# razayunus/ManhattanSLAM

Measured on AMD Instinct MI355X. Metric: RGB-D frames/sec at 640x480 (ORB+surfel front end), higher is better.
Workload: dtype u8/i32 (ORB)/f32+f64 (surfel)

## Files before the change

manhattanslam_amd/csrc/msl_orb.hip:

```cpp

#include "msl_orb_dev.h"

#include <type_traits>

#include <cfloat>
#include <cmath>
#include <cstdlib>

using namespace msl;
using namespace msl::orb;

namespace {

__constant__ int8_t c_pattern[1024] = {
#include "../../include/msl_orb_pattern.inc"
};

__device__ __forceinline__ const uint8_t *level_ptr(const OrbDev &P, int frame, int l, int &pitch) {
    if (l == 0) { pitch = (int)P.inRowStride; return P.in + (size_t)frame * P.inFrameStride; }
    pitch = P.lv[l].pitch;
    return P.pyr + (size_t)frame * P.pyrStride + P.lv[l].off;
}

__device__ __forceinline__ bool xcd_item(int nx, int ny, int &x, int &y) {
    const unsigned g = blockIdx.x, C = gridDim.x >> 3;
    const unsigned v = (g & 7u) * C + (g >> 3);
    if (v >= (unsigned)nx * (unsigned)ny) return false;
    x = (int)(v % (unsigned)nx); y = (int)(v / (unsigned)nx);
    return true;
}
inline unsigned xcd_grid1(long long items) { return (unsigned)(8 * ((items + 7) / 8)); }

__global__ __launch_bounds__(256) void k_resize(OrbDev P, int l) {
    const int frame = blockIdx.z;
    const LevelDev &D = P.lv[l];
    const int dx = blockIdx.x * 64 + (threadIdx.x & 63);
    const int dy = blockIdx.y * 4 + (threadIdx.x >> 6);
    if (dx >= D.w || dy >= D.h) return;
    int sp;
    const uint8_t *src = level_ptr(P, frame, l - 1, sp);
    const ResizeTap tx = P.taps[D.xtabOff + dx], ty = P.taps[D.ytabOff + dy];
    const uint8_t *r0 = src + (size_t)ty.s0 * sp, *r1 = src + (size_t)ty.s1 * sp;
    const int h0 = r0[tx.s0] * tx.c0 + r0[tx.s1] * tx.c1;
    const int h1 = r1[tx.s0] * tx.c0 + r1[tx.s1] * tx.c1;
    int v = (((ty.c0 * (h0 >> 4)) >> 16) + ((ty.c1 * (h1 >> 4)) >> 16) + 2) >> 2;
    v = min(max(v, 0), 255);
    P.pyr[(size_t)frame * P.pyrStride + D.off + (size_t)dy * D.pitch + dx] = (uint8_t)v;
}

__global__ __launch_bounds__(256) void k_pyramid(OrbDev P) {
    extern __shared__ uint8_t s_pyr[];
    int tileI, frame;
    if (!xcd_item(P.pyrTX * P.pyrTY, P.nFrames, tileI, frame)) return;
    const int ti = tileI % P.pyrTX, tj = tileI / P.pyrTX;
    const int L = P.nlevels;
    PyrRange rx = P.pyrX[ti], ry = P.pyrY[tj];
    int sx0 = rx.needLo, sy0 = ry.needLo, sw = rx.needHi - rx.needLo, sh = ry.needHi - ry.needLo;
    int spitch = (sw + 3) & ~3;
    {
        int pitch;
        const uint8_t *img = level_ptr(P, frame, 0, pitch);
        const int nw = spitch >> 2, imgW = P.lv[0].w;
        const unsigned m = ((1u << 22) + nw - 1) / nw;
        for (int i = threadIdx.x; i < nw * sh; i += 256) {
            const int r = (int)__umulhi((unsigned)i << 10, m), q = i - r * nw;
            const int x = sx0 + 4 * q;
            const uint8_t *src = img + (unsigned)((sy0 + r) * pitch + x);
            unsigned v = 0;
            if (x + 3 < imgW) __builtin_memcpy(&v, src, 4);
            else
                for (int e = 0; e < 4 && x + e < imgW; e++) v |= (unsigned)src[e] << (8 * e);
            reinterpret_cast<unsigned *>(s_pyr)[i] = v;
        }
    }
    __syncthreads();
    for (int l = 1; l < L; l++) {
        const LevelDev &D = P.lv[l];
        const uint8_t *src = s_pyr + (((l - 1) & 1) ? P.pyrBuf0 : 0u);
        uint8_t *dst = s_pyr + ((l & 1) ? P.pyrBuf0 : 0u);
        rx = P.pyrX[l * P.pyrTX + ti]; ry = P.pyrY[l * P.pyrTY + tj];
        const int dx0 = rx.needLo, dy0 = ry.needLo, dw = rx.needHi - rx.needLo, dh = ry.needHi - ry.needLo;
        uint8_t *out = P.pyr + (size_t)frame * P.pyrStride + D.off;
        const unsigned m = ((1u << 22) + dw - 1) / dw;
        for (int i = threadIdx.x; i < dw * dh; i += 256) {
            const int r = (int)__umulhi((unsigned)i << 10, m), c = i - r * dw;
            const int dx = dx0 + c, dy = dy0 + r;
            const ResizeTap tx = P.taps[D.xtabOff + dx], ty = P.taps[D.ytabOff + dy];
            const uint8_t *r0 = src + (ty.s0 - sy0) * spitch - sx0, *r1 = src + (ty.s1 - sy0) * spitch - sx0;
            const int h0 = r0[tx.s0] * tx.c0 + r0[tx.s1] * tx.c1;
            const int h1 = r1[tx.s0] * tx.c0 + r1[tx.s1] * tx.c1;
            int v = (((ty.c0 * (h0 >> 4)) >> 16) + ((ty.c1 * (h1 >> 4)) >> 16) + 2) >> 2;
            v = min(max(v, 0), 255);
            dst[i] = (uint8_t)v;
            if (dx >= rx.ownLo && dx < rx.ownHi && dy >= ry.ownLo && dy < ry.ownHi) out[(size_t)dy * D.pitch + dx] = (uint8_t)v;
        }
        sx0 = dx0; sy0 = dy0; sw = dw; sh = dh; spitch = dw;
        __syncthreads();
    }
}

typedef short s16x2 __attribute__((ext_vector_type(2)));
__device__ __forceinline__ s16x2 pk_min(s16x2 a, s16x2 b) { return __builtin_elementwise_min(a, b); }
__device__ __forceinline__ s16x2 pk_max(s16x2 a, s16x2 b) { return __builtin_elementwise_max(a, b); }
__device__ __forceinline__ int fast_score16(const uint8_t *t, int tp) {
    const int v = t[0];
    const int ring[16] = {t[3 * tp], t[3 * tp + 1], t[2 * tp + 2], t[tp + 3], t[3], t[-tp + 3], t[-2 * tp + 2], t[-3 * tp + 1],
                          t[-3 * tp], t[-3 * tp - 1], t[-2 * tp - 2], t[-tp - 3], t[-3], t[tp - 3], t[2 * tp - 2], t[3 * tp - 1]};
    s16x2 x[16], lo2[16], lo4[16];
#pragma unroll
    for (int k = 0; k < 16; k++) { const int d = v - ring[k]; x[k] = (s16x2){(short)d, (short)-d}; }
#pragma unroll
    for (int k = 0; k < 16; k++) lo2[k] = pk_min(x[k], x[(k + 1) & 15]);
#pragma unroll
    for (int k = 0; k < 16; k++) lo4[k] = pk_min(lo2[k], lo2[(k + 2) & 15]);
    s16x2 a = (s16x2){(short)-256, (short)-256};
#pragma unroll
    for (int k = 0; k < 16; k++) a = pk_max(a, pk_min(pk_min(lo4[k], lo4[(k + 4) & 15]), x[(k + 8) & 15]));
    return max((int)a.x, (int)a.y) - 1;
}

__device__ __forceinline__ bool fast_candidate(const uint8_t *t, int tp, int th) {
    const int v = t[0];
    const int d0 = v - t[3 * tp], d8 = v - t[-3 * tp], d4 = v - t[3], d12 = v - t[-3];
    const int d2 = v - t[2 * tp + 2], d10 = v - t[-2 * tp - 2], d6 = v - t[-2 * tp + 2], d14 = v - t[2 * tp - 2];
    const bool bright = (d0 > th || d8 > th) && (d4 > th || d12 > th) && (d2 > th || d10 > th) && (d6 > th || d14 > th);
    const bool dark = (d0 < -th || d8 < -th) && (d4 < -th || d12 < -th) && (d2 < -th || d10 < -th) && (d6 < -th || d14 < -th);
    return bright || dark;
}

__global__ __launch_bounds__(256) void k_fast(OrbDev P) {
    __shared__ __attribute__((aligned(4))) uint8_t s_tile[(MAXCELL + 6) * (MAXCELL + 8)];
    __shared__ __attribute__((aligned(4))) uint8_t s_score[(MAXCELL + 2) * (MAXCELL + 2)];
    __shared__ unsigned s_bits[2][MAXCELL * MAXCELL / 32];
    __shared__ unsigned short s_list[MAXCELL * MAXCELL];
    __shared__ unsigned s_wave[17];
    __shared__ unsigned s_cnt[3];

    int cellI, frame;
    if (!xcd_item(P.cellsPerFrame, P.nFrames, cellI, frame)) return;
    const CellDev C = P.cells[cellI];
    const int tid = threadIdx.x;
    uint32_t *cnt_out = P.cellCnt + (size_t)frame * P.cellsPerFrame + cellI;
    const int cw = C.cw, ch = C.ch;
    if (cw <= 0 || ch <= 0) { if (tid == 0) *cnt_out = 0; return; }
    int pitch;
    const uint8_t *img = level_ptr(P, frame, C.level, pitch);

    const int tw = cw + 6, th = ch + 6, tp = (tw + 3) & ~3;
    const unsigned mCw = ((1u << 20) + cw - 1) / cw;
    {
        const int nw = tp >> 2;
        const unsigned mNw = ((1u << 20) + nw - 1) / nw;
        const uint8_t *src = img + (size_t)(C.y0 - 3) * pitch + (C.x0 - 3);
        for (int i = tid; i < nw * th; i += 256) {
            const int r = (int)(((unsigned)i * mNw) >> 20), q = i - r * nw;
            uint32_t w4;
            __builtin_memcpy(&w4, src + (size_t)r * pitch + 4 * q, 4);
            *reinterpret_cast<uint32_t *>(&s_tile[r * tp + 4 * q]) = w4;
        }
    }
    const int sp = cw + 2;
    for (int i = tid; i < (sp * (ch + 2) + 3) >> 2; i += 256) reinterpret_cast<uint32_t *>(s_score)[i] = 0u;
    if (tid < MAXCELL * MAXCELL / 32) { s_bits[0][tid] = 0; s_bits[1][tid] = 0; }
    if (tid < 3) s_cnt[tid] = 0;
    __syncthreads();
    const int npx = cw * ch;
    const int thQuick = min(P.iniTh, P.minTh);
    for (int i0 = 0; i0 < npx; i0 += 256) {
        const int i = i0 + tid;
        bool cand = false;
        if (i < npx) {
            const int r = (int)(((unsigned)i * mCw) >> 20), c = i - r * cw;
            cand = fast_candidate(&s_tile[(r + 3) * tp + c + 3], tp, thQuick);
        }
        const unsigned long long m = __ballot(cand);
        if (m) {
            unsigned base = 0;
            if ((tid & 63) == 0) base = atomicAdd(&s_cnt[2], (unsigned)__popcll(m));
            base = (unsigned)__builtin_amdgcn_readlane((int)base, 0);
            if (cand) s_list[base + __popcll(m & ((1ull << (tid & 63)) - 1ull))] = (unsigned short)i;
        }
    }
    __syncthreads();
    const int nlist = (int)s_cnt[2];
    for (int j = tid; j < nlist; j += 256) {
        const int i = s_list[j];
        const int r = (int)(((unsigned)i * mCw) >> 20), c = i - r * cw;
        const int s = fast_score16(&s_tile[(r + 3) * tp + c + 3], tp);
        s_score[(r + 1) * sp + c + 1] = (uint8_t)max(s, 0);
    }
    __syncthreads();
    unsigned c_ini = 0, c_min = 0;
    for (int j = tid; j < nlist; j += 256) {
        const int i = s_list[j];
        const int r = (int)(((unsigned)i * mCw) >> 20), c = i - r * cw;
        const uint8_t *q = &s_score[(r + 1) * sp + c + 1];
        const int s = q[0];
        if (s < thQuick) continue;
        const bool lm = s > q[-1] && s > q[1] && s > q[-sp - 1] && s > q[-sp] && s > q[-sp + 1] &&
                        s > q[sp - 1] && s > q[sp] && s > q[sp + 1];
        if (!lm) continue;
        if (s >= P.iniTh) { atomicOr(&s_bits[0][i >> 5], 1u << (i & 31)); c_ini++; }
        if (s >= P.minTh) { atomicOr(&s_bits[1][i >> 5], 1u << (i & 31)); c_min++; }
    }
    if (c_ini) atomicAdd(&s_cnt[0], c_ini);
    if (c_min) atomicAdd(&s_cnt[1], c_min);
    __syncthreads();
    const int sel = s_cnt[0] ? 0 : 1;
    const unsigned total = s_cnt[0] ? s_cnt[0] : s_cnt[1];
    if (tid == 0) *cnt_out = total;
    if (total == 0) return;
    uint32_t *out = P.cellKeys + (size_t)frame * P.keysPerFrame + C.keyOff;
    static_assert(MAXCELL * MAXCELL / 32 <= 256, "one bitmap word per thread");
    unsigned word = tid < MAXCELL * MAXCELL / 32 ? s_bits[sel][tid] : 0u;
    unsigned tot;
    unsigned pos = block_excl_scan((unsigned)__popc(word), s_wave, &tot);
    while (word) {
        const int i = tid * 32 + __builtin_ctz(word);
        word &= word - 1;
        const int r = (int)(((unsigned)i * mCw) >> 20), c = i - r * cw;
        const unsigned kx = C.x0 + c - 16, ky = C.y0 + r - 16;
        out[pos++] = kx | (ky << 12) | ((unsigned)s_score[(r + 1) * sp + c + 1] << 24);
    }
}

struct Rect { short x0, y0, x1, y1; };

__device__ __forceinline__ int quadrant(const Rect r, int x, int y) {
    const int mx = r.x0 + ((r.x1 - r.x0 + 1) >> 1), my = r.y0 + ((r.y1 - r.y0 + 1) >> 1);
    return (x < mx ? 0 : 1) + (y < my ? 0 : 2);
}
__device__ __forceinline__ Rect child_rect(const Rect r, int q) {
    const short mx = r.x0 + ((r.x1 - r.x0 + 1) >> 1), my = r.y0 + ((r.y1 - r.y0 + 1) >> 1);
    Rect c;
    c.x0 = (q & 1) ? mx : r.x0; c.x1 = (q & 1) ? r.x1 : mx;
    c.y0 = (q & 2) ? my : r.y0; c.y1 = (q & 2) ? r.y1 : my;
    return c;
}

#ifdef MSL_OCT_STAMPS
#define OCT_STAMP(P, level, frame, idx)                                                                                   \
    do {                                                                                                                  \
        const int i_ = (idx);                                                                                             \
        if ((level) == 0 && (frame) == 0 && threadIdx.x == 0 && i_ < 100) {                                               \
            unsigned long long *d_ = reinterpret_cast<unsigned long long *>(reinterpret_cast<unsigned char *>((P).err) + 128); \
            d_[2 * i_] = __builtin_amdgcn_s_memrealtime(); d_[2 * i_ + 1] = __builtin_amdgcn_s_memtime();                 \
        }                                                                                                                 \
    } while (0)
#else
#define OCT_STAMP(P, level, frame, idx) do { } while (0)
#endif
template <int KPT> struct OctKeys {
    static constexpr bool REG = KPT > 0;
    static constexpr int OCT_KPT = KPT > 0 ? KPT : 1;
    uint32_t key[OCT_KPT];
    unsigned node[OCT_KPT], quad[OCT_KPT];
    uint32_t *gkeys; uint16_t *gnode; unsigned n; int tid;
    unsigned per;
    template <typename F> __device__ __forceinline__ void for_each(F f) {
        if constexpr (REG) {
#pragma unroll
            for (int j = 0; j < OCT_KPT; j++) {
                const unsigned k = (unsigned)tid * per + (unsigned)j;
                if ((unsigned)j < per && k < n) f(k, key[j], node[j], quad[j]);
            }
        } else {
            for (unsigned k = tid; k < n; k += OCT_NT) {
                unsigned nd = gnode[k], q = 0xFFFFFFFFu;
                const unsigned nd0 = nd;
                f(k, gkeys[k], nd, q);
                if (nd != nd0) gnode[k] = (uint16_t)nd;
            }
        }
    }
};

template <int KPT>
__device__ __forceinline__ void octree_body(const OrbDev &P, const LevelDev &G, OctKeys<KPT> &K, unsigned char *s_dyn, unsigned *s_wave, int *s_misc, int frame,
                                            int level) {
    constexpr bool REG = KPT > 0;
    constexpr int OCT_KPT = KPT > 0 ? KPT : 1;
    const int M = P.maxNode, tid = threadIdx.x, N = G.quota;
    const unsigned n = K.n;
    Rect *const s_rectB = reinterpret_cast<Rect *>(s_dyn);
    unsigned *const s_cntB = reinterpret_cast<unsigned *>(s_rectB + 2 * M);
    unsigned *const s_cc = s_cntB + 2 * M;
    short *const s_crankB = reinterpret_cast<short *>(s_cc + 4 * M);
    unsigned *const s_FG = reinterpret_cast<unsigned *>(s_crankB + 2 * M);
    unsigned short *const s_L = reinterpret_cast<unsigned short *>(s_FG + 4 * M);
    unsigned short *const s_order = s_L + M;
    unsigned short *const s_rankOf = s_order + M;
    int *nsel = P.nsel + frame * P.nlevels + level;
    uint32_t *sel = P.sel + ((size_t)frame * P.nlevels + level) * P.selCap;

    const unsigned lane = (unsigned)tid & 63u;
    auto hist_add = [&](unsigned *ctr, unsigned q) {
        unsigned long long todo = __ballot(q != 0xFFFFFFFFu);
        while (todo) {
            const unsigned leader = (unsigned)__builtin_ctzll(todo);
            const unsigned qq = (unsigned)__builtin_amdgcn_readlane((int)q, (int)leader);
            const unsigned long long mm = __ballot(q == qq);
            if (lane == leader) atomicAdd(&ctr[qq], (unsigned)__popcll(mm));
            todo &= ~mm;
        }
    };
    auto for_each_hist = [&](unsigned *ctr, auto f) {
// ... 571 lines not shown
    unsigned w = nib | ((unsigned)__builtin_amdgcn_update_dpp(0, (int)nib, 0x101, 0xF, 0xF, true) << 4);
    w |= (unsigned)__builtin_amdgcn_update_dpp(0, (int)w, 0x102, 0xF, 0xF, true) << 8;
    w |= (unsigned)__builtin_amdgcn_update_dpp(0, (int)w, 0x104, 0xF, 0xF, true) << 16;
    msl_keypoint *kp = P.kps + (size_t)frame * P.outCap + outIdx;
    uint32_t *dsc = (uint32_t *)(P.desc + ((size_t)frame * P.outCap + outIdx) * 32);
    if ((lane & 7) == 0) dsc[lane >> 3] = w;
    if (lane == 0) {
        float fx = (float)x, fy = (float)y;
        if (level != 0) { fx *= D.scale; fy *= D.scale; }
        kp->x = fx; kp->y = fy; kp->size = (float)D.patch; kp->angle = angle;
        kp->response = (float)score; kp->octave = level; kp->class_id = -1;
        if (P.frameOn) {
            const size_t o = (size_t)frame * P.outCap + outIdx;
            float ux = fx, uy = fy;
            if (P.fp.k1 != 0.0) undistort_point(P.fp, fx, fy, &ux, &uy);
            P.unXY[2 * o] = ux; P.unXY[2 * o + 1] = uy;
            const float d = *(const float *)((const uint8_t *)P.depth + (size_t)frame * P.depthFrameStride + (size_t)(int)fy * P.depthRowStride +
                                             sizeof(float) * (size_t)(int)fx);
            P.depthOut[o] = d > 0 ? d : -1.0f;
            P.uRight[o] = d > 0 ? ux - P.fp.bf / d : -1.0f;
            const int posX = (int)roundf((ux - P.fp.minX) * P.gridWInv), posY = (int)roundf((uy - P.fp.minY) * P.gridHInv);
            P.gridCell[o] = (posX < 0 || posX >= MSL_FRAME_GRID_COLS || posY < 0 || posY >= MSL_FRAME_GRID_ROWS) ? -1 : posX * MSL_FRAME_GRID_ROWS + posY;
        }
    }
}

const char *kKernelNames[MSL_ORB_NKERNELS] = {"k_pyramid", "k_fast", "k_octree", "k_blur", "k_describe", "copy"};

}

namespace msl {
namespace orb {

const char *kernel_name(int kid) { return kKernelNames[kid]; }

int allow_octree_lds(int octLds) {
    if (octLds <= 32 * 1024) return MSL_OK;
    MSL_HIP_TRY(hipFuncSetAttribute(reinterpret_cast<const void *>(k_octree<16>), hipFuncAttributeMaxDynamicSharedMemorySize, octLds));
    MSL_HIP_TRY(hipFuncSetAttribute(reinterpret_cast<const void *>(k_octree<32>), hipFuncAttributeMaxDynamicSharedMemorySize, octLds));
    return MSL_OK;
}

}
}

int orb_launch_pipeline(const OrbDev *dev, OrbLaunch *launch, const uint8_t *d_gray, size_t rowStride, size_t frameStride, int n,
                        msl_keypoint *d_kps, uint8_t *d_desc, int *d_nout, const FrameEpilogue *ep) {
    OrbLaunch &q = *launch;
    OrbDev P = *dev;
    P.in = d_gray; P.inRowStride = rowStride; P.inFrameStride = frameStride;
    P.kps = d_kps; P.desc = d_desc; P.nout = d_nout;
    P.frameOn = ep ? 1 : 0;
    P.nFrames = n;
    if (ep) {
        P.fp = ep->fp;
        P.gridWInv = (float)MSL_FRAME_GRID_COLS / (float)(ep->fp.maxX - ep->fp.minX);
        P.gridHInv = (float)MSL_FRAME_GRID_ROWS / (float)(ep->fp.maxY - ep->fp.minY);
        P.depth = ep->depth; P.depthRowStride = ep->depthRowStride; P.depthFrameStride = ep->depthFrameStride;
        P.unXY = ep->unXY; P.depthOut = ep->depthOut; P.uRight = ep->uRight; P.gridCell = ep->gridCell;
    }
    hipStream_t s = q.stream;
    const int L = P.nlevels;
    static const bool perLevel = getenv("MSL_ORB_PYRAMID") && !strcmp(getenv("MSL_ORB_PYRAMID"), "levels");
    if (P.pyrTX && !perLevel) {
        q.prof.begin(KID_RESIZE, s);
        hipLaunchKernelGGL(k_pyramid, dim3(xcd_grid1((long long)P.pyrTX * P.pyrTY * n)), dim3(256), q.pyrLds, s, P);
        q.prof.end(s);
    } else {
        for (int l = 1; l < L; l++) {
            const LevelDev &G = P.lv[l];
            q.prof.begin(KID_RESIZE, s);
            hipLaunchKernelGGL(k_resize, dim3((G.w + 63) / 64, (G.h + 3) / 4, n), dim3(256), 0, s, P, l);
            q.prof.end(s);
        }
    }
    const bool fork = n == 1 && q.sideStream && !q.prof.on;
    if (fork) {
        MSL_HIP_TRY(hipEventRecord(q.evFork, s));
        MSL_HIP_TRY(hipStreamWaitEvent(q.sideStream, q.evFork, 0));
        hipLaunchKernelGGL(k_blur, dim3(xcd_grid1((long long)P.blurTiles * n)), dim3(256), 0, q.sideStream, P);
        MSL_HIP_TRY(hipEventRecord(q.evJoin, q.sideStream));
    }
    q.prof.begin(KID_FAST, s);
    hipLaunchKernelGGL(k_fast, dim3(xcd_grid1((long long)P.cellsPerFrame * n)), dim3(256), 0, s, P);
    q.prof.end(s);
    q.prof.begin(KID_OCTREE, s);
    if (q.octBig) hipLaunchKernelGGL(k_octree<32>, dim3(xcd_grid1((long long)L * n)), dim3(OCT_NT), (size_t)P.octLds, s, P);
    else hipLaunchKernelGGL(k_octree<16>, dim3(xcd_grid1((long long)L * n)), dim3(OCT_NT), (size_t)P.octLds, s, P);
    q.prof.end(s);
    if (fork) {
        MSL_HIP_TRY(hipStreamWaitEvent(s, q.evJoin, 0));
    } else {
        q.prof.begin(KID_BLUR, s);
        hipLaunchKernelGGL(k_blur, dim3(xcd_grid1((long long)P.blurTiles * n)), dim3(256), 0, s, P);
        q.prof.end(s);
    }
    q.prof.begin(KID_DESCRIBE, s);
    hipLaunchKernelGGL(k_describe, dim3(xcd_grid1((long long)((P.selCap + 3) / 4) * L * n)), dim3(256), 0, s, P);
    q.prof.end(s);
    MSL_HIP_TRY(hipGetLastError());
    return MSL_OK;
}
```

manhattanslam_amd/csrc/msl_orb_dev.h:

```cpp
#pragma once

#include "msl_common.h"

namespace msl {
namespace orb {

constexpr int ML = 12;
constexpr int MAXCELL = 64;
constexpr int MAXNODE = 1024;
constexpr int OCT_NT = 512;
constexpr int OCT_NODE_BYTES = 66;
constexpr int BT_W = 64, BT_H = 32;

struct FrameEpilogue {
    msl_frame_params fp; const float *depth; size_t depthRowStride, depthFrameStride;
    float *unXY, *depthOut, *uRight; int *gridCell;
};

enum { KID_RESIZE = 0, KID_FAST, KID_OCTREE, KID_BLUR, KID_DESCRIBE, KID_COPY };
const char *kernel_name(int kid);

struct OrbLaunch {
    hipStream_t stream = nullptr;
    hipStream_t sideStream = nullptr; hipEvent_t evFork = nullptr, evJoin = nullptr;
    KernelProfiler prof;
    size_t pyrLds = 0;
    bool octBig = false;
};

int allow_octree_lds(int octLds);

}
}

namespace {

struct LevelDev {
    int w, h, pitch;
    unsigned off;
    unsigned boff;
    int nCols, nRows, wCell, hCell;
    int cellBase, nCells;
    int keyBase, keyCap;
    int quota;
    int nIni; float hX;
    float scale; int patch;
    unsigned xtabOff, ytabOff;
    int tileBase, tilesX, tilesY;
};

struct CellDev {
    short level, x0, y0, cw, ch, _pad;
    unsigned keyOff;
};

struct ResizeTap { short s0, s1, c0, c1; };
struct PyrRange { short ownLo, ownHi, needLo, needHi; };

struct OrbDev {
    int nlevels, iniTh, minTh;
    int cellsPerFrame, keysPerFrame, selCap, outCap, blurTiles;
    unsigned long long pyrStride, blurStride;
    LevelDev lv[msl::orb::ML];
    int umax[16];
    const uint8_t *in; unsigned long long inRowStride, inFrameStride;
    uint8_t *pyr, *blur;
    const CellDev *cells;
    const ResizeTap *taps;
    const PyrRange *pyrX, *pyrY;
    int pyrTX, pyrTY; unsigned pyrBuf0;
    uint32_t *cellCnt, *cellKeys, *keys;
    uint16_t *knode;
    uint32_t *sel; int *nsel, *ncand;
    msl_keypoint *kps; uint8_t *desc; int *nout; int *err;
    int frameOn;
    msl_frame_params fp; float gridWInv, gridHInv;
    const float *depth; unsigned long long depthRowStride, depthFrameStride;
    float *unXY, *depthOut, *uRight; int *gridCell;
    int nFrames;
    int maxNode;
    int octLds;
};

}

extern "C" int orb_launch_pipeline(const OrbDev *dev, msl::orb::OrbLaunch *q, const uint8_t *d_gray, size_t rowStride, size_t frameStride, int n,
                                       msl_keypoint *d_kps, uint8_t *d_desc, int *d_nout, const msl::orb::FrameEpilogue *ep);
```

manhattanslam_amd/csrc/msl_orb_host.hip:

```cpp

#include "msl_orb_dev.h"

#include <algorithm>
#include <cmath>
#include <memory>
#include <vector>

using namespace msl;
using namespace msl::orb;

namespace {

inline int cv_round_f(float v) { return (int)lrintf(v); }
inline int cv_round_d(double v) { return (int)lrint(v); }
inline int cv_floor_d(double v) { int i = (int)v; return i - (i > v); }
inline int cv_ceil_d(double v) { int i = (int)v; return i + (i < v); }

}

struct OrbConfig {
    int nfeatures = 0, nlevels = 0, iniTh = 0, minTh = 0, maxBatch = 0;
    int outCap = 0;
    std::vector<float> scale, invScale;
    std::vector<int> perLevel;
    int umax[16];
};

struct msl_orb : OrbConfig, OrbLaunch {
    int device = 0;
    int maxW = 0, maxH = 0;
    double scaleFactor = 0;
    std::vector<float> sigma2, invSigma2;
    int geomW = 0, geomH = 0;
    OrbDev dev{};
    bool ownStream = true;
    struct Geometry { DevBuf in, pyr, blur, cells, taps, pyrRanges, cellCnt, cellKeys, keys, knode, sel, nsel, ncand, outBlock; } geo;
    size_t inPitch = 0, outKpsOff = 0, outDescOff = 0;
    msl_keypoint *d_kps = nullptr; uint8_t *d_desc = nullptr; int *d_nout = nullptr;
    DevBuf d_err; PinBuf h_err;
    PinBuf h_pinIn, h_pinOut;
    DevBuf d_depthIn;
    DevBuf d_unXY, d_depthOut, d_uRight, d_gridCell;
    int lastFrames = 0;
};

namespace {

struct OrbPlan {
    int W = 0, H = 0;
    OrbDev dev{};
    std::vector<CellDev> cells;
    std::vector<ResizeTap> taps;
    std::vector<PyrRange> pyrX, pyrY;
    size_t pyrLds = 0, inPitch = 0, outKpsOff = 0, outDescOff = 0;
    int needCap = 0, outCap = 0;
    bool octBig = false;
    size_t pyrOff = 0, blurOff = 0;
    unsigned keyOff = 0;
    int tileBase = 0, maxList = 0, maxSel = 0;
};

int plan_level_grid(const OrbConfig *h, OrbPlan &P, int l) {
    LevelDev &G = P.dev.lv[l];
    const float s = h->invScale[l];
    G.w = cv_round_f((float)P.W * s); G.h = cv_round_f((float)P.H * s);
    G.pitch = (G.w + 63) & ~63;
    G.scale = h->scale[l];
    G.patch = (int)(31 * h->scale[l]);
    G.quota = h->perLevel[l];
    if (l > 0) { G.off = (unsigned)P.pyrOff; P.pyrOff += (size_t)G.pitch * G.h; }
    G.boff = (unsigned)P.blurOff; P.blurOff += (size_t)G.pitch * G.h;
    const int minB = 16, maxBX = G.w - 16, maxBY = G.h - 16;
    const float width = (float)(maxBX - minB), height = (float)(maxBY - minB);
    const float Wc = 30;
    G.nCols = (int)(width / Wc); G.nRows = (int)(height / Wc);
    if (G.nCols < 1 || G.nRows < 1) {
        set_error("level %d (%dx%d) is too small for the 30-px FAST grid", l, G.w, G.h);
        return MSL_ERR_INVALID;
    }
    G.wCell = (int)ceilf(width / G.nCols); G.hCell = (int)ceilf(height / G.nRows);
    if (G.wCell > MAXCELL || G.hCell > MAXCELL || G.w > 4095 + 16 || G.h > 4095 + 16) {
        set_error("unsupported level geometry %dx%d (cell %dx%d)", G.w, G.h, G.wCell, G.hCell);
        return MSL_ERR_INVALID;
    }
    G.cellBase = (int)P.cells.size(); G.nCells = G.nRows * G.nCols;
    G.keyBase = (int)P.keyOff;
    for (int i = 0; i < G.nRows; i++)
        for (int j = 0; j < G.nCols; j++) {
            const float iniY = (float)(minB + i * G.hCell), iniX = (float)(minB + j * G.wCell);
            float maxY = iniY + G.hCell + 6, maxX = iniX + G.wCell + 6;
            CellDev c{}; c.level = (short)l; c.keyOff = P.keyOff;
            const bool skip = (iniY >= maxBY - 3) || (iniX >= maxBX - 6);
            if (maxY > maxBY) maxY = (float)maxBY;
            if (maxX > maxBX) maxX = (float)maxBX;
            const int cw = (int)maxX - (int)iniX - 6, chh = (int)maxY - (int)iniY - 6;
            if (!skip && cw > 0 && chh > 0) {
                c.x0 = (short)((int)iniX + 3); c.y0 = (short)((int)iniY + 3); c.cw = (short)cw; c.ch = (short)chh;
                P.keyOff += (unsigned)(((cw + 1) / 2) * ((chh + 1) / 2));
            }
            P.cells.push_back(c);
        }
    G.keyCap = (int)P.keyOff - G.keyBase;
    if (G.keyCap >= (1 << 24)) { set_error("level too large"); return MSL_ERR_INVALID; }
    G.tilesX = (G.w + BT_W - 1) / BT_W; G.tilesY = (G.h + BT_H - 1) / BT_H;
    G.tileBase = P.tileBase; P.tileBase += G.tilesX * G.tilesY;
    return MSL_OK;
}

int plan_level_quadtree(OrbPlan &P, int l) {
    LevelDev &G = P.dev.lv[l];
    const int minB = 16, maxBX = G.w - 16, maxBY = G.h - 16;
    G.nIni = (int)roundf((float)(maxBX - minB) / (maxBY - minB));
    if (G.nIni < 1) { set_error("unsupported aspect ratio (nIni = 0)"); return MSL_ERR_INVALID; }
    G.hX = (float)(maxBX - minB) / G.nIni;
    if (std::max(G.quota, 4 * G.nIni) + 2 > MAXNODE) { set_error("per-level quota %d exceeds %d", G.quota, MAXNODE - 2); return MSL_ERR_INVALID; }
    P.maxList = std::max(P.maxList, std::max(G.quota, 4 * G.nIni) + 2);
    P.needCap += std::max(G.quota + 2, 4 * G.nIni); P.maxSel = std::max(P.maxSel, std::max(G.quota + 2, 4 * G.nIni));
    return MSL_OK;
}

void plan_level_taps(OrbPlan &P, int l) {
    LevelDev &G = P.dev.lv[l];
    std::vector<ResizeTap> &taps = P.taps;
    const int sw = P.dev.lv[l - 1].w, sh = P.dev.lv[l - 1].h;
    const double scale_x = 1. / ((double)G.w / sw), scale_y = 1. / ((double)G.h / sh);
    G.xtabOff = (unsigned)taps.size();
    for (int dx = 0; dx < G.w; dx++) {
        float fx = (float)((dx + 0.5) * scale_x - 0.5);
        int sx = cv_floor_d(fx);
        fx -= sx;
        if (sx < 0) { fx = 0; sx = 0; }
        if (sx >= sw - 1) { fx = 0; sx = sw - 1; }
        ResizeTap t;
        t.s0 = (short)sx; t.s1 = (short)std::min(sx + 1, sw - 1);
        t.c0 = (short)std::min(std::max(cv_round_f((1.f - fx) * 2048), -32768), 32767);
        t.c1 = (short)std::min(std::max(cv_round_f(fx * 2048), -32768), 32767);
        if (sx + 1 >= sw) { t.c0 = 2048; t.c1 = 0; }
        taps.push_back(t);
    }
    G.ytabOff = (unsigned)taps.size();
    for (int dy = 0; dy < G.h; dy++) {
        float fy = (float)((dy + 0.5) * scale_y - 0.5);
        int sy = cv_floor_d(fy);
        fy -= sy;
        ResizeTap t;
        t.s0 = (short)std::min(std::max(sy, 0), sh - 1); t.s1 = (short)std::min(std::max(sy + 1, 0), sh - 1);
        t.c0 = (short)std::min(std::max(cv_round_f((1.f - fy) * 2048), -32768), 32767);
        t.c1 = (short)std::min(std::max(cv_round_f(fy * 2048), -32768), 32767);
        taps.push_back(t);
    }
}

void plan_pyramid(OrbPlan &P) {
    OrbDev &D = P.dev;
    const int L = D.nlevels;
    const std::vector<ResizeTap> &taps = P.taps;
    D.pyrTX = D.pyrTY = 0;
    if (L < 2) return;
    const int TX = std::max(1, D.lv[L - 1].w / 22), TY = std::max(1, D.lv[L - 1].h / 22);
    auto axis = [&](int T, bool isX, std::vector<PyrRange> &out, std::vector<int> &extent) {
        out.assign((size_t)L * T, PyrRange{0, 0, 0, 0});
        extent.assign(L, 0);
        for (int i = 0; i < T; i++) {
            for (int l = 1; l < L; l++) {
                const int n = isX ? D.lv[l].w : D.lv[l].h;
                PyrRange &r = out[(size_t)l * T + i];
                r.ownLo = (short)((long long)i * n / T); r.ownHi = (short)((long long)(i + 1) * n / T);
// ... 19 lines not shown
    size_t b0 = 0, b1 = 0;
    bool ok = true;
    for (int l = 0; l < L; l++) {
        const size_t a = (size_t)(l == 0 ? (ex[l] + 3) & ~3 : ex[l]) * ey[l];
        if (l & 1) b1 = std::max(b1, a); else b0 = std::max(b0, a);
        if (l >= 1 && (D.lv[l].w < TX || D.lv[l].h < TY)) ok = false;
    }
    b0 = (b0 + 15) & ~(size_t)15;
    for (int l = 0; l < L; l++) if (ex[l] >= 128 || (size_t)ex[l] * ey[l] >= (1u << 15)) ok = false;
    if (ok && b0 + b1 <= 48 * 1024) { D.pyrTX = TX; D.pyrTY = TY; D.pyrBuf0 = (unsigned)b0; P.pyrLds = b0 + b1; }
}

int plan_geometry(const OrbConfig *h, int W, int H, OrbPlan &P) {
    P.W = W; P.H = H;
    OrbDev &D = P.dev;
    const int L = h->nlevels, B = h->maxBatch;
    D.nlevels = L; D.iniTh = h->iniTh; D.minTh = h->minTh;
    for (int i = 0; i < 16; i++) D.umax[i] = h->umax[i];
    for (int l = 0; l < L; l++) {
        int rc = plan_level_grid(h, P, l);
        if (rc == MSL_OK) rc = plan_level_quadtree(P, l);
        if (rc != MSL_OK) return rc;
        if (l > 0) plan_level_taps(P, l);
    }
    plan_pyramid(P);
    D.cellsPerFrame = (int)P.cells.size();
    D.keysPerFrame = (int)P.keyOff;
    D.selCap = P.maxSel;
    D.maxNode = ((P.maxList + 63) & ~63) + 64;
    {
        int maxCells = 0;
        for (int l = 0; l < L; l++) maxCells = std::max(maxCells, D.lv[l].nCells);
        D.octLds = (int)((std::max<size_t>((size_t)OCT_NODE_BYTES * D.maxNode, 2 * sizeof(unsigned) * (size_t)(maxCells + 1)) + 15) & ~(size_t)15);
    }
    P.outCap = h->outCap ? h->outCap : std::max(h->nfeatures + 2 * L, P.needCap);
    if (P.needCap > P.outCap) {
        set_error("frame %dx%d can return %d keypoints (aspect ratio: %d quadtree roots), the extractor was created for %d; create it with this frame size", W, H,
                  P.needCap, D.lv[0].nIni, P.outCap);
        return MSL_ERR_INVALID;
    }
    D.outCap = P.outCap;
    P.octBig = (long long)W * H > 640ll * 480 * 3 / 2;
    D.blurTiles = P.tileBase;
    D.pyrStride = (P.pyrOff + 255) & ~(size_t)255;
    D.blurStride = (P.blurOff + 255) & ~(size_t)255;
    P.inPitch = (size_t)((W + 63) & ~63);
    P.outKpsOff = (sizeof(int) * (size_t)B + 255) & ~(size_t)255;
    P.outDescOff = P.outKpsOff + ((sizeof(msl_keypoint) * (size_t)D.outCap * B + 255) & ~(size_t)255);
    return MSL_OK;
}

int commit_geometry(msl_orb *h, const OrbPlan &P) {
    MSL_HIP_TRY(hipStreamSynchronize(h->stream));
    h->geomW = h->geomH = 0;
    msl_orb::Geometry &g = h->geo;
    g = msl_orb::Geometry();
    OrbDev &D = h->dev;
    D = P.dev;
    const size_t B = (size_t)h->maxBatch, L = (size_t)D.nlevels, nCells = P.cells.size(), nKeys = P.keyOff;
    MSL_HIP_TRY(grow_all(h->stream, {{g.in, P.inPitch * P.H * B}, {g.pyr, std::max<size_t>(D.pyrStride, 256) * B}, {g.blur, D.blurStride * B},
                                     {g.cells, sizeof(CellDev) * nCells}, {g.taps, sizeof(ResizeTap) * std::max<size_t>(P.taps.size(), 1)},
                                     {g.pyrRanges, D.pyrTX ? sizeof(PyrRange) * (P.pyrX.size() + P.pyrY.size()) : 0},
                                     {g.cellCnt, sizeof(uint32_t) * nCells * B}, {g.cellKeys, sizeof(uint32_t) * nKeys * B},
                                     {g.keys, sizeof(uint32_t) * nKeys * B}, {g.knode, sizeof(uint16_t) * nKeys * B},
                                     {g.sel, sizeof(uint32_t) * (size_t)D.selCap * L * B}, {g.nsel, sizeof(int) * L * B}, {g.ncand, sizeof(int) * L * B},
                                     {g.outBlock, P.outDescOff + (size_t)32 * D.outCap * B}}));
    MSL_HIP_TRY(hipMemcpy(g.cells.p, P.cells.data(), sizeof(CellDev) * nCells, hipMemcpyHostToDevice));
    if (!P.taps.empty())
        MSL_HIP_TRY(hipMemcpy(g.taps.p, P.taps.data(), sizeof(ResizeTap) * P.taps.size(), hipMemcpyHostToDevice));
    if (D.pyrTX) {
        PyrRange *ranges = (PyrRange *)g.pyrRanges.p;
        MSL_HIP_TRY(hipMemcpy(ranges, P.pyrX.data(), sizeof(PyrRange) * P.pyrX.size(), hipMemcpyHostToDevice));
        MSL_HIP_TRY(hipMemcpy(ranges + P.pyrX.size(), P.pyrY.data(), sizeof(PyrRange) * P.pyrY.size(), hipMemcpyHostToDevice));
        D.pyrX = ranges; D.pyrY = ranges + P.pyrX.size();
    }
    D.pyr = (uint8_t *)g.pyr.p; D.blur = (uint8_t *)g.blur.p; D.cells = (const CellDev *)g.cells.p; D.taps = (const ResizeTap *)g.taps.p;
    D.cellCnt = (uint32_t *)g.cellCnt.p; D.cellKeys = (uint32_t *)g.cellKeys.p; D.keys = (uint32_t *)g.keys.p; D.knode = (uint16_t *)g.knode.p;
    D.sel = (uint32_t *)g.sel.p; D.nsel = (int *)g.nsel.p; D.ncand = (int *)g.ncand.p; D.err = (int *)h->d_err.p;
    uint8_t *out = (uint8_t *)g.outBlock.p;
    h->d_nout = reinterpret_cast<int *>(out);
    h->d_kps = reinterpret_cast<msl_keypoint *>(out + P.outKpsOff);
    h->d_desc = out + P.outDescOff;
    h->outCap = P.outCap; h->inPitch = P.inPitch; h->outKpsOff = P.outKpsOff; h->outDescOff = P.outDescOff;
    h->pyrLds = P.pyrLds; h->octBig = P.octBig;
    { const int rc = allow_octree_lds(D.octLds); if (rc != MSL_OK) return rc; }
    h->geomW = P.W; h->geomH = P.H;
    return MSL_OK;
}

int ensure_geometry(msl_orb *h, int W, int H) {
    if (h->geomW == W && h->geomH == H) return MSL_OK;
    OrbPlan plan;
    const int rc = plan_geometry(h, W, H, plan);
    return rc != MSL_OK ? rc : commit_geometry(h, plan);
}

int check_device_error(msl_orb *h) {
    MSL_HIP_TRY(hipMemcpyAsync(h->h_err.p, h->d_err.p, sizeof(int), hipMemcpyDeviceToHost, h->stream));
    MSL_HIP_TRY(hipStreamSynchronize(h->stream));
    h->prof.drain();
    const int e = *(const int *)h->h_err.p;
    if (e) {
        (void)hipMemsetAsync(h->d_err.p, 0, sizeof(int), h->stream);
        set_error("device-side bound exceeded in ORB pipeline (code %d)", e);
        return MSL_ERR_OVERFLOW;
    }
    return MSL_OK;
}

struct GrayOnDevice { const uint8_t *p; size_t rowStride, frameStride; };

int stage_gray(msl_orb *h, const uint8_t *gray, int n, int W, int H, size_t rowStride, size_t frameStride, msl_mem mem, GrayOnDevice &out) {
    out = {gray, rowStride, frameStride};
    if (mem != MSL_MEM_HOST) return MSL_OK;
    uint8_t *d_in = (uint8_t *)h->geo.in.p;
    h->prof.begin(KID_COPY, h->stream);
    if (rowStride == (size_t)W && h->inPitch == (size_t)W && frameStride == (size_t)W * H) {
        MSL_HIP_TRY(hipMemcpyAsync(d_in, gray, (size_t)W * H * n, hipMemcpyHostToDevice, h->stream));
    } else {
        for (int f = 0; f < n; f++)
            MSL_HIP_TRY(hipMemcpy2DAsync(d_in + (size_t)f * h->inPitch * H, h->inPitch, gray + (size_t)f * frameStride, rowStride, W, H, hipMemcpyHostToDevice, h->stream));
    }
    h->prof.end(h->stream);
    out = {d_in, h->inPitch, h->inPitch * H};
    return MSL_OK;
}

struct OutArray { void *user; void *own; size_t bytesPerKey; };

int run_batch(msl_orb *h, const GrayOnDevice &g, int n, FrameEpilogue *ep, const OutArray *outs, int nOuts, int cap, int32_t *n_out, msl_mem out_mem) {
    const int outCap = h->outCap;
    const bool direct = out_mem == MSL_MEM_DEVICE && cap == outCap;
    void *dst[6];
    for (int i = 0; i < nOuts; i++) dst[i] = direct ? outs[i].user : outs[i].own;
    if (ep) { ep->unXY = (float *)dst[2]; ep->depthOut = (float *)dst[3]; ep->uRight = (float *)dst[4]; ep->gridCell = (int *)dst[5]; }
    const int rc = orb_launch_pipeline(&h->dev, h, g.p, g.rowStride, g.frameStride, n, (msl_keypoint *)dst[0], (uint8_t *)dst[1], direct ? n_out : h->d_nout, ep);
    if (rc != MSL_OK) return rc;
    h->lastFrames = n;
    if (direct) return MSL_OK;
    const hipMemcpyKind kind = out_mem == MSL_MEM_HOST ? hipMemcpyDeviceToHost : hipMemcpyDeviceToDevice;
    MSL_HIP_TRY(hipMemcpyAsync(n_out, h->d_nout, sizeof(int) * n, kind, h->stream));
    for (int i = 0; i < nOuts; i++) {
        const size_t b = outs[i].bytesPerKey;
        MSL_HIP_TRY(hipMemcpy2DAsync(outs[i].user, b * cap, outs[i].own, b * outCap, b * outCap, n, kind, h->stream));
    }
    return out_mem == MSL_MEM_HOST ? check_device_error(h) : MSL_OK;
}

}

extern "C" {

msl_orb *msl_orb_create(int nfeatures, float scaleFactorF, int nlevels, int iniThFAST, int minThFAST, int max_width,
                        int max_height, int max_batch, int device) noexcept {
    try {
    if (nfeatures < 1 || nlevels < 1 || nlevels > ML || !(scaleFactorF > 1.0f) || iniThFAST < 1 || iniThFAST > 255 ||
        minThFAST < 1 || minThFAST > 255 || max_width < 1 || max_height < 1 || max_batch < 1) {
        set_error("msl_orb_create: invalid argument");
        return nullptr;
    }
    if (bind_device(device) != MSL_OK) return nullptr;
    std::unique_ptr<msl_orb, void (*)(msl_orb *)> guard(new msl_orb, [](msl_orb *p) { msl_orb_destroy(p); });
    msl_orb *h = guard.get();
    h->device = device; h->nfeatures = nfeatures; h->nlevels = nlevels; h->iniTh = iniThFAST; h->minTh = minThFAST;
    h->maxW = max_width; h->maxH = max_height; h->maxBatch = max_batch;
    h->scaleFactor = scaleFactorF;
    h->scale.resize(nlevels); h->sigma2.resize(nlevels); h->invScale.resize(nlevels); h->invSigma2.resize(nlevels);
// ... 340 lines not shown
```

Measured before the change: 25860.

## Rewrite FAST cell kernel as single-wave with packed 4-pixel prefilter

The FAST corner kernel now runs one 64-lane wavefront per cell instead of 256 threads. This replaces block barriers with wave-level fences and sizes dynamic LDS to the actual cell geometry. The candidate prefilter tests four pixels at once with packed 16-bit min/max on 32-bit word loads. Keys are emitted directly via ballot/mbcnt compaction instead of shared bitmaps plus a block scan. The minTh fallback is now a second pass run only when no keypoint passes iniTh, which trades less parallelism per cell for lower sync, LDS and occupancy overhead.

```diff
diff --git a/manhattanslam_amd/csrc/msl_orb.hip b/manhattanslam_amd/csrc/msl_orb.hip
--- a/manhattanslam_amd/csrc/msl_orb.hip
+++ b/manhattanslam_amd/csrc/msl_orb.hip
@@ -1,5 +1,6 @@
 
 #include "msl_orb_dev.h"
+#include "msl_orb_fast.h"
 
 #include <type_traits>
 
@@ -99,129 +100,117 @@
     }
 }
 
-typedef short s16x2 __attribute__((ext_vector_type(2)));
-__device__ __forceinline__ s16x2 pk_min(s16x2 a, s16x2 b) { return __builtin_elementwise_min(a, b); }
-__device__ __forceinline__ s16x2 pk_max(s16x2 a, s16x2 b) { return __builtin_elementwise_max(a, b); }
-__device__ __forceinline__ int fast_score16(const uint8_t *t, int tp) {
-    const int v = t[0];
-    const int ring[16] = {t[3 * tp], t[3 * tp + 1], t[2 * tp + 2], t[tp + 3], t[3], t[-tp + 3], t[-2 * tp + 2], t[-3 * tp + 1],
-                          t[-3 * tp], t[-3 * tp - 1], t[-2 * tp - 2], t[-tp - 3], t[-3], t[tp - 3], t[2 * tp - 2], t[3 * tp - 1]};
-    s16x2 x[16], lo2[16], lo4[16];
-#pragma unroll
-    for (int k = 0; k < 16; k++) { const int d = v - ring[k]; x[k] = (s16x2){(short)d, (short)-d}; }
-#pragma unroll
-    for (int k = 0; k < 16; k++) lo2[k] = pk_min(x[k], x[(k + 1) & 15]);
-#pragma unroll
-    for (int k = 0; k < 16; k++) lo4[k] = pk_min(lo2[k], lo2[(k + 2) & 15]);
-    s16x2 a = (s16x2){(short)-256, (short)-256};
-#pragma unroll
-    for (int k = 0; k < 16; k++) a = pk_max(a, pk_min(pk_min(lo4[k], lo4[(k + 4) & 15]), x[(k + 8) & 15]));
-    return max((int)a.x, (int)a.y) - 1;
-}
-
-__device__ __forceinline__ bool fast_candidate(const uint8_t *t, int tp, int th) {
-    const int v = t[0];
-    const int d0 = v - t[3 * tp], d8 = v - t[-3 * tp], d4 = v - t[3], d12 = v - t[-3];
-    const int d2 = v - t[2 * tp + 2], d10 = v - t[-2 * tp - 2], d6 = v - t[-2 * tp + 2], d14 = v - t[2 * tp - 2];
-    const bool bright = (d0 > th || d8 > th) && (d4 > th || d12 > th) && (d2 > th || d10 > th) && (d6 > th || d14 > th);
-    const bool dark = (d0 < -th || d8 < -th) && (d4 < -th || d12 < -th) && (d2 < -th || d10 < -th) && (d6 < -th || d14 < -th);
-    return bright || dark;
-}
-
-__global__ __launch_bounds__(256) void k_fast(OrbDev P) {
-    __shared__ __attribute__((aligned(4))) uint8_t s_tile[(MAXCELL + 6) * (MAXCELL + 8)];
-    __shared__ __attribute__((aligned(4))) uint8_t s_score[(MAXCELL + 2) * (MAXCELL + 2)];
-    __shared__ unsigned s_bits[2][MAXCELL * MAXCELL / 32];
-    __shared__ unsigned short s_list[MAXCELL * MAXCELL];
-    __shared__ unsigned s_wave[17];
-    __shared__ unsigned s_cnt[3];
-
+__device__ __forceinline__ void wave_lds_sync() {
+    __builtin_amdgcn_fence(__ATOMIC_RELEASE, "wavefront");
+    __builtin_amdgcn_wave_barrier();
+    __builtin_amdgcn_fence(__ATOMIC_ACQUIRE, "wavefront");
+}
+__device__ __forceinline__ unsigned lanes_below(unsigned long long m, unsigned add = 0) {
+    return __builtin_amdgcn_mbcnt_hi((unsigned)(m >> 32), __builtin_amdgcn_mbcnt_lo((unsigned)m, add));
+}
+
+__global__ __launch_bounds__(64) void k_fast(OrbDev P) {
+    extern __shared__ __attribute__((aligned(16))) uint8_t s_fast[];
     int cellI, frame;
     if (!xcd_item(P.cellsPerFrame, P.nFrames, cellI, frame)) return;
     const CellDev C = P.cells[cellI];
-    const int tid = threadIdx.x;
+    const int lane = threadIdx.x;
     uint32_t *cnt_out = P.cellCnt + (size_t)frame * P.cellsPerFrame + cellI;
     const int cw = C.cw, ch = C.ch;
-    if (cw <= 0 || ch <= 0) { if (tid == 0) *cnt_out = 0; return; }
+    if (cw <= 0 || ch <= 0) { if (lane == 0) *cnt_out = 0; return; }
     int pitch;
     const uint8_t *img = level_ptr(P, frame, C.level, pitch);
-
-    const int tw = cw + 6, th = ch + 6, tp = (tw + 3) & ~3;
-    const unsigned mCw = ((1u << 20) + cw - 1) / cw;
+    const FastLds F = fast_lds(cw, ch);
+    const int tp = F.tp, sp = F.sp;
+    uint8_t *const s_tile = s_fast;
+    uint8_t *const s_score = s_fast + F.scoreOff;
+    unsigned short *const s_list = reinterpret_cast<unsigned short *>(s_fast + F.listOff);
+
     {
-        const int nw = tp >> 2;
+        const int nw = (cw + 6 + 3) >> 2;
         const unsigned mNw = ((1u << 20) + nw - 1) / nw;
         const uint8_t *src = img + (size_t)(C.y0 - 3) * pitch + (C.x0 - 3);
-        for (int i = tid; i < nw * th; i += 256) {
+        for (int i = lane; i < nw * (ch + 6); i += 64) {
             const int r = (int)(((unsigned)i * mNw) >> 20), q = i - r * nw;
             uint32_t w4;
             __builtin_memcpy(&w4, src + (size_t)r * pitch + 4 * q, 4);
             *reinterpret_cast<uint32_t *>(&s_tile[r * tp + 4 * q]) = w4;
         }
     }
-    const int sp = cw + 2;
-    for (int i = tid; i < (sp * (ch + 2) + 3) >> 2; i += 256) reinterpret_cast<uint32_t *>(s_score)[i] = 0u;
-    if (tid < MAXCELL * MAXCELL / 32) { s_bits[0][tid] = 0; s_bits[1][tid] = 0; }
-    if (tid < 3) s_cnt[tid] = 0;
-    __syncthreads();
-    const int npx = cw * ch;
-    const int thQuick = min(P.iniTh, P.minTh);
-    for (int i0 = 0; i0 < npx; i0 += 256) {
-        const int i = i0 + tid;
-        bool cand = false;
-        if (i < npx) {
-            const int r = (int)(((unsigned)i * mCw) >> 20), c = i - r * cw;
-            cand = fast_candidate(&s_tile[(r + 3) * tp + c + 3], tp, thQuick);
-        }
-        const unsigned long long m = __ballot(cand);
-        if (m) {
-            unsigned base = 0;
-            if ((tid & 63) == 0) base = atomicAdd(&s_cnt[2], (unsigned)__popcll(m));
-            base = (unsigned)__builtin_amdgcn_readlane((int)base, 0);
-            if (cand) s_list[base + __popcll(m & ((1ull << (tid & 63)) - 1ull))] = (unsigned short)i;
-        }
-    }
-    __syncthreads();
-    const int nlist = (int)s_cnt[2];
-    for (int j = tid; j < nlist; j += 256) {
-        const int i = s_list[j];
-        const int r = (int)(((unsigned)i * mCw) >> 20), c = i - r * cw;
-        const int s = fast_score16(&s_tile[(r + 3) * tp + c + 3], tp);
-        s_score[(r + 1) * sp + c + 1] = (uint8_t)max(s, 0);
-    }
-    __syncthreads();
-    unsigned c_ini = 0, c_min = 0;
-    for (int j = tid; j < nlist; j += 256) {
-        const int i = s_list[j];
-        const int r = (int)(((unsigned)i * mCw) >> 20), c = i - r * cw;
-        const uint8_t *q = &s_score[(r + 1) * sp + c + 1];
-        const int s = q[0];
-        if (s < thQuick) continue;
-        const bool lm = s > q[-1] && s > q[1] && s > q[-sp - 1] && s > q[-sp] && s > q[-sp + 1] &&
-                        s > q[sp - 1] && s > q[sp] && s > q[sp + 1];
-        if (!lm) continue;
-        if (s >= P.iniTh) { atomicOr(&s_bits[0][i >> 5], 1u << (i & 31)); c_ini++; }
-        if (s >= P.minTh) { atomicOr(&s_bits[1][i >> 5], 1u << (i & 31)); c_min++; }
-    }
-    if (c_ini) atomicAdd(&s_cnt[0], c_ini);
-    if (c_min) atomicAdd(&s_cnt[1], c_min);
-    __syncthreads();
-    const int sel = s_cnt[0] ? 0 : 1;
-    const unsigned total = s_cnt[0] ? s_cnt[0] : s_cnt[1];
-    if (tid == 0) *cnt_out = total;
-    if (total == 0) return;
+    for (int i = lane; i < (sp * (ch + 2) + 3) >> 2; i += 64) reinterpret_cast<uint32_t *>(s_score)[i] = 0u;
+    wave_lds_sync();
+
+    const int ngr = (cw + 3) >> 2, nGroups = ngr * ch, wp = tp >> 2;
+    const unsigned mG = ((1u << 20) + ngr - 1) / ngr;
     uint32_t *out = P.cellKeys + (size_t)frame * P.keysPerFrame + C.keyOff;
-    static_assert(MAXCELL * MAXCELL / 32 <= 256, "one bitmap word per thread");
-    unsigned word = tid < MAXCELL * MAXCELL / 32 ? s_bits[sel][tid] : 0u;
-    unsigned tot;
-    unsigned pos = block_excl_scan((unsigned)__popc(word), s_wave, &tot);
-    while (word) {
-        const int i = tid * 32 + __builtin_ctz(word);
-        word &= word - 1;
-        const int r = (int)(((unsigned)i * mCw) >> 20), c = i - r * cw;
-        const unsigned kx = C.x0 + c - 16, ky = C.y0 + r - 16;
-        out[pos++] = kx | (ky << 12) | ((unsigned)s_score[(r + 1) * sp + c + 1] << 24);
-    }
+
+    auto stage = [&](int thQuick, int thKeep) -> unsigned {
+        unsigned nlist = 0;
+        for (int g0 = 0; g0 < nGroups; g0 += 64) {
+            const int g = g0 + lane;
+            unsigned m4 = 0;
+            int r = 0, c0 = 0;
+            if (g < nGroups) {
+                r = (int)(((unsigned)g * mG) >> 20); c0 = 4 * (g - r * ngr);
+                const uint32_t *w = reinterpret_cast<const uint32_t *>(s_tile + r * tp + c0);
+                const uint32_t u0 = w[0], u1 = w[1];
+                const uint32_t a0 = w[wp], a1 = w[wp + 1], a2 = w[wp + 2];
+                const uint32_t b0 = w[3 * wp], b1 = w[3 * wp + 1], b2 = w[3 * wp + 2];
+                const uint32_t d0 = w[5 * wp], d1 = w[5 * wp + 1], d2 = w[5 * wp + 2];
+                const uint32_t e0 = w[6 * wp], e1 = w[6 * wp + 1];
+                m4 = fast_quick4(fast_bytes(b0, b1, 3),  fast_bytes(e0, e1, 3),  fast_bytes(u0, u1, 3),  fast_bytes(b1, b2, 2),  b0,
+                                  fast_bytes(d1, d2, 1),  fast_bytes(a0, a1, 1),  fast_bytes(a1, a2, 1),  fast_bytes(d0, d1, 1), thQuick);
+                if (cw - c0 < 4) m4 &= (1u << (cw - c0)) - 1u;
+            }
+            const unsigned long long q0 = __ballot(m4 & 1u), q1 = __ballot(m4 & 2u), q2 = __ballot(m4 & 4u), q3 = __ballot(m4 & 8u);
+            if (q0 | q1 | q2 | q3) {
+                unsigned pos = nlist + lanes_below(q3, lanes_below(q2, lanes_below(q1, lanes_below(q0))));
+                const unsigned rc = ((unsigned)r << 8) | (unsigned)c0;
+                if (m4 & 1u) s_list[pos++] = (unsigned short)rc;
+                if (m4 & 2u) s_list[pos++] = (unsigned short)(rc + 1);
+                if (m4 & 4u) s_list[pos++] = (unsigned short)(rc + 2);
+                if (m4 & 8u) s_list[pos++] = (unsigned short)(rc + 3);
+                nlist += (unsigned)(__popcll(q0) + __popcll(q1) + __popcll(q2) + __popcll(q3));
+            }
+        }
+        wave_lds_sync();
+        for (unsigned j = lane; j < nlist; j += 64) {
+            const unsigned rc = s_list[j];
+            const int r = (int)(rc >> 8), c = (int)(rc & 255u);
+            const uint8_t *t = &s_tile[(r + 3) * tp + c + 3];
+            const int ring[16] = {t[3 * tp], t[3 * tp + 1], t[2 * tp + 2], t[tp + 3], t[3], t[-tp + 3], t[-2 * tp + 2], t[-3 * tp + 1],
+                                  t[-3 * tp], t[-3 * tp - 1], t[-2 * tp - 2], t[-tp - 3], t[-3], t[tp - 3], t[2 * tp - 2], t[3 * tp - 1]};
+            s_score[(r + 1) * sp + c + 1] = (uint8_t)max(fast_score16((int)t[0], ring), 0);
+        }
+        wave_lds_sync();
+        unsigned kept = 0;
+        for (unsigned j0 = 0; j0 < nlist; j0 += 64) {
+            const unsigned j = j0 + lane;
+            bool keep = false;
+            uint32_t key = 0;
+            if (j < nlist) {
+                const unsigned rc = s_list[j];
+                const int r = (int)(rc >> 8), c = (int)(rc & 255u);
+                const uint8_t *q = &s_score[(r + 1) * sp + c + 1];
+                const int s = q[0];
+                keep = s >= thKeep && s > q[-1] && s > q[1] && s > q[-sp - 1] && s > q[-sp] && s > q[-sp + 1] && s > q[sp - 1] && s > q[sp] && s > q[sp + 1];
+                const unsigned kx = C.x0 + c - 16, ky = C.y0 + r - 16;
+                key = kx | (ky << 12) | ((unsigned)s << 24);
+            }
+            const unsigned long long m = __ballot(keep);
+            if (keep) out[kept + lanes_below(m)] = key;
+            kept += (unsigned)__popcll(m);
+        }
+        return kept;
+    };
+
+    const int thIni = min(P.iniTh, 256), thMin = min(P.minTh, 256);
+    unsigned total = stage(thIni, thIni);
+    if (total == 0) {
+        wave_lds_sync();
+        total = stage(min(thIni, thMin), thMin);
+    }
+    if (lane == 0) *cnt_out = total;
 }
 
 struct Rect { short x0, y0, x1, y1; };
@@ -959,7 +948,7 @@
         MSL_HIP_TRY(hipEventRecord(q.evJoin, q.sideStream));
     }
     q.prof.begin(KID_FAST, s);
-    hipLaunchKernelGGL(k_fast, dim3(xcd_grid1((long long)P.cellsPerFrame * n)), dim3(256), 0, s, P);
+    hipLaunchKernelGGL(k_fast, dim3(xcd_grid1((long long)P.cellsPerFrame * n)), dim3(64), q.fastLds, s, P);
     q.prof.end(s);
     q.prof.begin(KID_OCTREE, s);
     if (q.octBig) hipLaunchKernelGGL(k_octree<32>, dim3(xcd_grid1((long long)L * n)), dim3(OCT_NT), (size_t)P.octLds, s, P);
diff --git a/manhattanslam_amd/csrc/msl_orb_dev.h b/manhattanslam_amd/csrc/msl_orb_dev.h
--- a/manhattanslam_amd/csrc/msl_orb_dev.h
+++ b/manhattanslam_amd/csrc/msl_orb_dev.h
@@ -25,8 +25,19 @@
     hipStream_t sideStream = nullptr; hipEvent_t evFork = nullptr, evJoin = nullptr;
     KernelProfiler prof;
     size_t pyrLds = 0;
+    size_t fastLds = 0;
     bool octBig = false;
 };
+
+struct FastLds { int tp, sp, scoreOff, listOff, bytes; };
+__host__ __device__ inline FastLds fast_lds(int cw, int ch) {
+    FastLds f;
+    f.tp = 4 * ((cw + 3) >> 2) + 8; f.sp = cw + 2;
+    f.scoreOff = f.tp * (ch + 6);
+    f.listOff = (f.scoreOff + f.sp * (ch + 2) + 3) & ~3;
+    f.bytes = f.listOff + 2 * cw * ch;
+    return f;
+}
 
 int allow_octree_lds(int octLds);
 
diff --git a/manhattanslam_amd/csrc/msl_orb_fast.h b/manhattanslam_amd/csrc/msl_orb_fast.h
--- /dev/null
+++ b/manhattanslam_amd/csrc/msl_orb_fast.h
@@ -0,0 +1,75 @@
+#pragma once
+
+#include <stdint.h>
+
+#if defined(__HIPCC__)
+#define MSL_FAST_HD __host__ __device__ __forceinline__
+#define MSL_FAST_UNROLL _Pragma("unroll")
+#else
+#define MSL_FAST_HD inline
+#define MSL_FAST_UNROLL
+#endif
+
+namespace msl {
+namespace orb {
+
+#if defined(__HIP_DEVICE_COMPILE__)
+typedef short s16x2 __attribute__((ext_vector_type(2)));
+MSL_FAST_HD s16x2 pk_make(int lo, int hi) { return (s16x2){(short)lo, (short)hi}; }
+MSL_FAST_HD s16x2 pk_min(s16x2 a, s16x2 b) { return __builtin_elementwise_min(a, b); }
+MSL_FAST_HD s16x2 pk_max(s16x2 a, s16x2 b) { return __builtin_elementwise_max(a, b); }
+MSL_FAST_HD s16x2 pk_add(s16x2 a, s16x2 b) { return a + b; }
+MSL_FAST_HD s16x2 pk_sub(s16x2 a, s16x2 b) { return a - b; }
+MSL_FAST_HD s16x2 pk_from_bits(uint32_t w) { return __builtin_bit_cast(s16x2, w); }
+MSL_FAST_HD uint32_t pk_bits(s16x2 a) { return __builtin_bit_cast(uint32_t, a); }
+#else
+struct s16x2 { short x, y; };
+MSL_FAST_HD s16x2 pk_make(int lo, int hi) { s16x2 r; r.x = (short)lo; r.y = (short)hi; return r; }
+MSL_FAST_HD s16x2 pk_min(s16x2 a, s16x2 b) { return pk_make(a.x < b.x ? a.x : b.x, a.y < b.y ? a.y : b.y); }
+MSL_FAST_HD s16x2 pk_max(s16x2 a, s16x2 b) { return pk_make(a.x > b.x ? a.x : b.x, a.y > b.y ? a.y : b.y); }
+MSL_FAST_HD s16x2 pk_add(s16x2 a, s16x2 b) { return pk_make(a.x + b.x, a.y + b.y); }
+MSL_FAST_HD s16x2 pk_sub(s16x2 a, s16x2 b) { return pk_make(a.x - b.x, a.y - b.y); }
+MSL_FAST_HD s16x2 pk_from_bits(uint32_t w) { return pk_make((int)(int16_t)(w & 0xFFFFu), (int)(int16_t)(w >> 16)); }
+MSL_FAST_HD uint32_t pk_bits(s16x2 a) { return (uint32_t)(uint16_t)a.x | ((uint32_t)(uint16_t)a.y << 16); }
+#endif
+
+MSL_FAST_HD s16x2 fast_pair(uint32_t w, int half) {
+    const uint32_t h = half ? w >> 16 : w;
+    return pk_from_bits((h & 0xFFu) | ((h & 0xFF00u) << 8));
+}
+
+MSL_FAST_HD uint32_t fast_bytes(uint32_t lo, uint32_t hi, int n) { return (lo >> (8 * n)) | (hi << (32 - 8 * n)); }
+
+MSL_FAST_HD unsigned fast_quick4(uint32_t c, uint32_t r0, uint32_t r8, uint32_t r4, uint32_t r12, uint32_t r2, uint32_t r10, uint32_t r6,
+                                 uint32_t r14, int th) {
+    const s16x2 t = pk_make(th, th);
+    uint32_t sign[2];
+    MSL_FAST_UNROLL
+    for (int half = 0; half < 2; half++) {
+        const s16x2 v = fast_pair(c, half);
+        const s16x2 a0 = fast_pair(r0, half), a8 = fast_pair(r8, half), a4 = fast_pair(r4, half), a12 = fast_pair(r12, half);
+        const s16x2 a2 = fast_pair(r2, half), a10 = fast_pair(r10, half), a6 = fast_pair(r6, half), a14 = fast_pair(r14, half);
+        const s16x2 lo = pk_max(pk_max(pk_min(a0, a8), pk_min(a4, a12)), pk_max(pk_min(a2, a10), pk_min(a6, a14)));
+        const s16x2 hi = pk_min(pk_min(pk_max(a0, a8), pk_max(a4, a12)), pk_min(pk_max(a2, a10), pk_max(a6, a14)));
+        sign[half] = pk_bits(pk_sub(pk_add(lo, t), v)) | pk_bits(pk_sub(pk_add(v, t), hi));
+    }
+    return ((sign[0] >> 15) & 1u) | ((sign[0] >> 30) & 2u) | ((sign[1] >> 13) & 4u) | ((sign[1] >> 28) & 8u);
+}
+
+MSL_FAST_HD int fast_score16(int v, const int *ring) {
+    s16x2 x[16], lo2[16], lo4[16];
+    MSL_FAST_UNROLL
+    for (int k = 0; k < 16; k++) { const int d = v - ring[k]; x[k] = pk_make(d, -d); }
+    MSL_FAST_UNROLL
+    for (int k = 0; k < 16; k++) lo2[k] = pk_min(x[k], x[(k + 1) & 15]);
+    MSL_FAST_UNROLL
+    for (int k = 0; k < 16; k++) lo4[k] = pk_min(lo2[k], lo2[(k + 2) & 15]);
+    s16x2 a = pk_make(-256, -256);
+    MSL_FAST_UNROLL
+    for (int k = 0; k < 16; k++) a = pk_max(a, pk_min(pk_min(lo4[k], lo4[(k + 4) & 15]), x[(k + 8) & 15]));
+    const int p = a.x, n = a.y;
+    return (p > n ? p : n) - 1;
+}
+
+}
+}
diff --git a/manhattanslam_amd/csrc/msl_orb_host.hip b/manhattanslam_amd/csrc/msl_orb_host.hip
--- a/manhattanslam_amd/csrc/msl_orb_host.hip
+++ b/manhattanslam_amd/csrc/msl_orb_host.hip
@@ -52,7 +52,7 @@
     std::vector<CellDev> cells;
     std::vector<ResizeTap> taps;
     std::vector<PyrRange> pyrX, pyrY;
-    size_t pyrLds = 0, inPitch = 0, outKpsOff = 0, outDescOff = 0;
+    size_t pyrLds = 0, fastLds = 0, inPitch = 0, outKpsOff = 0, outDescOff = 0;
     int needCap = 0, outCap = 0;
     bool octBig = false;
     size_t pyrOff = 0, blurOff = 0;
@@ -83,6 +83,7 @@
         set_error("unsupported level geometry %dx%d (cell %dx%d)", G.w, G.h, G.wCell, G.hCell);
         return MSL_ERR_INVALID;
     }
+    P.fastLds = std::max(P.fastLds, (size_t)fast_lds(G.wCell, G.hCell).bytes);
     G.cellBase = (int)P.cells.size(); G.nCells = G.nRows * G.nCols;
     G.keyBase = (int)P.keyOff;
     for (int i = 0; i < G.nRows; i++)
@@ -268,7 +269,7 @@
     h->d_kps = reinterpret_cast<msl_keypoint *>(out + P.outKpsOff);
     h->d_desc = out + P.outDescOff;
     h->outCap = P.outCap; h->inPitch = P.inPitch; h->outKpsOff = P.outKpsOff; h->outDescOff = P.outDescOff;
-    h->pyrLds = P.pyrLds; h->octBig = P.octBig;
+    h->pyrLds = P.pyrLds; h->fastLds = P.fastLds; h->octBig = P.octBig;
     { const int rc = allow_octree_lds(D.octLds); if (rc != MSL_OK) return rc; }
     h->geomW = P.W; h->geomH = P.H;
     return MSL_OK;
```

After: 26430 (median of 6 runs). 2.2% higher.
